# fgvieira/ngsLD

Measured on AMD Instinct MI355X. Metric: SNP-pair EM-LD computations/sec @ n_ind=500, higher is better.
Workload: dtype f64

## Files before the change

include/ngsld.h:

```cpp
#ifndef NGSLD_H
#define NGSLD_H

#include <stddef.h>
#include <stdint.h>

#ifdef __cplusplus
extern "C" {
#endif

typedef struct ngsld_ctx ngsld_ctx;

enum {
  NGSLD_OK = 0,
  NGSLD_ERR_INVALID = -1,
  NGSLD_ERR_DEVICE = -2,
  NGSLD_ERR_NOMEM = -3,
  NGSLD_ERR_NAN = -4,
  NGSLD_ERR_MAF_RANGE = -5,
  NGSLD_ERR_SINK = -6,
  NGSLD_ERR_UNSUPPORTED = -7
};

typedef struct {
  uint64_t max_kb_dist;
// ... 79 lines not shown
int ngsld_set_replay(ngsld_ctx *ctx, int enable);
int ngsld_replay_stats(ngsld_ctx *ctx, uint64_t *pairs, uint64_t *sites);

int ngsld_set_exact_store(ngsld_ctx *ctx, int mode);
typedef struct {
  uint64_t pairs_flagged;
  uint64_t pairs_replayed;
  uint64_t pairs_on_device;
  uint64_t pairs_on_host;
  uint64_t sites_reevaluated;
  int32_t exact_store;
  int32_t text_rows_patched;
  double exact_store_build_s;
  uint64_t sites_degenerate;
} ngsld_replay_stats_t;
int ngsld_replay_info(ngsld_ctx *ctx, ngsld_replay_stats_t *out);

int ngsld_run_device(ngsld_ctx *ctx, uint64_t s1_begin, uint64_t s1_end, void *d_std, void *d_ext, void *hip_stream);
int ngsld_finish_device(ngsld_ctx *ctx);

int ngsld_last_kernel_time(ngsld_ctx *ctx, double *total_ms, uint64_t *n_launches, uint64_t *n_pairs);

const char *ngsld_pair_kernel(const ngsld_ctx *ctx);
int ngsld_describe_dispatch(uint64_t n_ind, int ignore_miss_data, char *buf, size_t buf_len);

int ngsld_set_tuning(ngsld_ctx *ctx, uint32_t pairs_per_item, uint64_t batch_pairs);

int ngsld_selftest(ngsld_ctx *ctx);

int ngsld_selftest_format(ngsld_ctx *ctx, uint64_t n, const ngsld_rec_std *std, const ngsld_rec_ext *ext, const double *dist,
                          const double *maf1, const double *maf2, char *text, uint64_t text_cap, uint64_t *row_len,
                          int32_t *needs_host);
int ngsld_selftest_printed(ngsld_ctx *ctx, uint64_t n, const double *x, int32_t precision, int32_t weight_type,
                           double min_weight, int64_t *micro, int32_t *micro_ok, int64_t *label, int32_t *label_rc);

typedef struct {
  uint64_t row_begin, row_end;
  uint64_t site_end;
} ngsld_slab;

int ngsld_window_ends(const double *pos_dist, uint64_t n_sites, const ngsld_params *params, uint32_t *row_end);

int ngsld_plan_slabs(const double *pos_dist, uint64_t n_sites, const ngsld_params *params, uint64_t max_slab_sites,
                     ngsld_slab *slabs, uint64_t cap, uint64_t *n_slabs);

uint64_t ngsld_slab_sites_for_budget(uint64_t n_ind, uint64_t budget_bytes);
// ... 304 lines not shown
```

ngsld_amd/capi.py:

```python
from __future__ import annotations

import ctypes as C
import os
import subprocess

import numpy as np

PKG_DIR = os.path.dirname(os.path.abspath(__file__))
REPO_DIR = os.path.dirname(PKG_DIR)
LIB_PATH = os.environ.get("NGSLD_LIB") or os.path.join(PKG_DIR, "libngsld.so")
CLI_PATH = os.path.join(PKG_DIR, "bin", "ngsLD")

OK, ERR_INVALID, ERR_DEVICE, ERR_NOMEM, ERR_NAN, ERR_MAF_RANGE, ERR_SINK, ERR_UNSUPPORTED = 0, -1, -2, -3, -4, -5, -6, -7


class Params(C.Structure):
    _fields_ = [("max_kb_dist", C.c_uint64), ("max_snp_dist", C.c_uint64), ("min_maf", C.c_double),
                ("ignore_miss_data", C.c_int32), ("extend_out", C.c_int32), ("rnd_sample", C.c_double),
                ("seed", C.c_uint64), ("first_row", C.c_uint64)]


class GenoOpts(C.Structure):
    _fields_ = [("log_scale", C.c_int32), ("ignore_miss_data", C.c_int32), ("on_device", C.c_int32),
                ("text_semantics", C.c_int32), ("call_geno", C.c_int32), ("per_individual_only", C.c_int32),
# ... 31 lines not shown
    items = np.zeros(len(uniq), dtype=ITEM)
    items["s1"] = s1[first]
    items["s2_begin"] = s1[first] + 1 + chunk[first] * span
    items["first_record"] = first
    np.bitwise_or.at(items["mask"], inv, np.uint64(1) << (s2 - items["s2_begin"][inv]).astype(np.uint64))
    last = np.zeros(len(uniq), dtype=np.int64)
    np.maximum.at(last, inv, s2 - items["s2_begin"][inv].astype(np.int64))
    items["count"] = last + 1
    return items


SINK_FN = C.CFUNCTYPE(C.c_int, C.c_void_p, C.POINTER(Batch))
MULTI_SINK_FN = C.CFUNCTYPE(C.c_int, C.c_void_p, C.c_int, C.POINTER(Batch))
READ_FN = C.CFUNCTYPE(C.c_int, C.c_void_p, C.c_uint64, C.c_uint64, C.c_void_p)
SLAB = np.dtype([("row_begin", "<u8"), ("row_end", "<u8"), ("site_end", "<u8")])

SYMBOLS = [
    "ngsld_version", "ngsld_create", "ngsld_destroy", "ngsld_last_error", "ngsld_set_geno_raw",
    "ngsld_set_geno_raw_opts", "ngsld_set_geno_lkl",
    "ngsld_get_maf", "ngsld_set_pos_dist", "ngsld_plan", "ngsld_plan_rows", "ngsld_run", "ngsld_run_device", "ngsld_set_text_output",
    "ngsld_set_replay_source", "ngsld_set_replay_matrix", "ngsld_set_replay", "ngsld_replay_stats", "ngsld_finish_device",
    "ngsld_set_exact_store", "ngsld_replay_info",
    "ngsld_plan_parts", "ngsld_run_multi", "ngsld_multi_last_distribution", "ngsld_rccl_selftest",
    "ngsld_last_kernel_time", "ngsld_pair_kernel", "ngsld_describe_dispatch", "ngsld_set_tuning", "ngsld_selftest", "ngsld_selftest_format",
    "ngsld_selftest_printed", "ngsld_reserve_text_buffers",
    "ngsld_window_ends", "ngsld_plan_slabs", "ngsld_slab_sites_for_budget", "ngsld_sites_for_budget", "ngsld_streamed_replay_info", "ngsld_set_memory_budget", "ngsld_device_memory", "ngsld_run_streamed", "ngsld_run_streamed_text",
    "ngsld_host_read_geno_bin_range",
    "ngsld_host_set_threads", "ngsld_host_read_pos", "ngsld_host_pos_dist", "ngsld_host_label", "ngsld_host_free_pos", "ngsld_host_pos_slice",
    "ngsld_host_geno_size_ok", "ngsld_host_read_geno_bin", "ngsld_host_read_geno_text", "ngsld_host_format_header", "ngsld_host_format_pair",
    "ngsld_host_format_double", "ngsld_host_write_batch", "ngsld_host_replay_pair", "ngsld_host_missing_call_log",
    "ngsld_host_gz_open", "ngsld_host_gz_close",
    "ngsld_prune", "ngsld_host_prune_graph", "ngsld_host_prune_label",
    "ngsld_decay", "ngsld_decay_bins", "ngsld_host_decay_fit",
    "ngsld_blocks", "ngsld_blocks_sites", "ngsld_blocks_matrix", "ngsld_blocks_text",
    "ngsld_site_ld", "ngsld_site_ld_get",
    "ngsld_clusters", "ngsld_clusters_sites", "ngsld_clusters_table",
    "ngsld_grid", "ngsld_grid_cells", "ngsld_grid_chromosomes", "ngsld_grid_get",
    "ngsld_linked_pairs",
    "ngsld_scan", "ngsld_scan_get",
    "ngsld_analyze",
    "ngsld_partners", "ngsld_partners_info", "ngsld_partners_get",
]


class ReplayStats(C.Structure):
    _fields_ = [("pairs_flagged", C.c_uint64), ("pairs_replayed", C.c_uint64), ("pairs_on_device", C.c_uint64),
                ("pairs_on_host", C.c_uint64), ("sites_reevaluated", C.c_uint64), ("exact_store", C.c_int32),
# ... 186 lines not shown
        L.ngsld_get_maf.argtypes = [vp, vp]
        L.ngsld_set_pos_dist.argtypes = [vp, vp]
        L.ngsld_plan.argtypes = [vp, C.POINTER(Params), C.POINTER(u64)]
        L.ngsld_plan_rows.argtypes = [vp, C.POINTER(C.POINTER(C.c_uint64)), C.POINTER(C.POINTER(C.c_uint32))]
        L.ngsld_run.argtypes = [vp, u64, u64, SINK_FN, vp]
        L.ngsld_run_device.argtypes = [vp, u64, u64, vp, vp, vp]
        if hasattr(L, "ngsld_set_replay_source"):
            L.ngsld_set_replay_source.argtypes = [vp, READ_FN, vp]
            if hasattr(L, "ngsld_set_replay_matrix"):
                L.ngsld_set_replay_matrix.argtypes = [vp, vp]
            L.ngsld_set_replay.argtypes = [vp, C.c_int]
            L.ngsld_replay_stats.argtypes = [vp, C.POINTER(u64), C.POINTER(u64)]
        if hasattr(L, "ngsld_replay_info"):
            L.ngsld_set_exact_store.argtypes = [vp, C.c_int]
            L.ngsld_replay_info.argtypes = [vp, C.POINTER(ReplayStats)]
            L.ngsld_finish_device.argtypes = [vp]
        if hasattr(L, "ngsld_set_text_output"):
            L.ngsld_set_text_output.argtypes = [vp, C.POINTER(C.c_char_p), C.c_int]
        L.ngsld_last_kernel_time.argtypes = [vp, C.POINTER(dbl), C.POINTER(u64), C.POINTER(u64)]
        L.ngsld_set_tuning.argtypes = [vp, C.c_uint32, u64]
        if hasattr(L, "ngsld_pair_kernel"):
            L.ngsld_pair_kernel.argtypes = [vp]
            L.ngsld_pair_kernel.restype = C.c_char_p
        L.ngsld_selftest.argtypes = [vp]
        if hasattr(L, "ngsld_selftest_format"):
            L.ngsld_selftest_format.argtypes = [vp, u64, vp, vp, vp, vp, vp, C.c_char_p, u64, vp, C.POINTER(C.c_int32)]
            L.ngsld_selftest_printed.argtypes = [vp, u64, vp, C.c_int32, C.c_int32, dbl, vp, vp, vp, vp]
        L.ngsld_window_ends.argtypes = [vp, u64, C.POINTER(Params), vp]
        L.ngsld_plan_slabs.argtypes = [vp, u64, C.POINTER(Params), u64, vp, u64, C.POINTER(u64)]
        L.ngsld_slab_sites_for_budget.argtypes = [u64, u64]
        L.ngsld_slab_sites_for_budget.restype = u64
        if hasattr(L, "ngsld_sites_for_budget"):
            L.ngsld_sites_for_budget.argtypes = [u64, u64, C.c_int]
            L.ngsld_sites_for_budget.restype = u64
        L.ngsld_device_memory.argtypes = [C.c_int, C.POINTER(u64), C.POINTER(u64)]
        L.ngsld_run_streamed.argtypes = [C.c_int, u64, u64, vp, C.POINTER(Params), C.POINTER(GenoOpts), u64, READ_FN, vp,
                                         vp, SINK_FN, vp, C.POINTER(u64), C.POINTER(u64), C.c_char_p, C.c_size_t]
        if hasattr(L, "ngsld_run_multi"):
            L.ngsld_plan_parts.argtypes = [vp, u64, C.POINTER(Params), C.c_int, vp]
            L.ngsld_run_multi.argtypes = [C.POINTER(C.c_int), C.c_int, u64, u64, vp, C.POINTER(Params), C.POINTER(GenoOpts),
                                          vp, READ_FN, vp, vp, MULTI_SINK_FN, vp, C.POINTER(C.c_char_p), C.c_int,
                                          C.POINTER(u64), C.c_char_p, C.c_size_t]
        if hasattr(L, "ngsld_multi_last_distribution"):
            L.ngsld_multi_last_distribution.argtypes = []
        if hasattr(L, "ngsld_rccl_selftest"):
            L.ngsld_rccl_selftest.argtypes = [C.c_int, u64, C.c_char_p, C.c_size_t]
# ... 697 lines not shown
                fallbacks[0] += 1
            return 0

        self._check(self._L.ngsld_run(self._h, s1_begin, s1_end, SINK_FN(sink), None))
        return b"".join(parts), fallbacks[0]

    def run_discard(self, s1_begin: int = 0, s1_end: int | None = None) -> int:
        s1_end = self.n_sites if s1_end is None else s1_end
        total = [0]

        def sink(_user, bp):
            total[0] += bp.contents.n_pairs
            return 0

        self._check(self._L.ngsld_run(self._h, s1_begin, s1_end, SINK_FN(sink), None))
        return total[0]

    def run_device(self, s1_begin: int, s1_end: int, d_std: int, d_ext: int | None, stream: int | None = None) -> None:
        self._check(self._L.ngsld_run_device(self._h, s1_begin, s1_end, d_std, d_ext, stream))

    def pair_kernel(self) -> str:
        return self._L.ngsld_pair_kernel(self._h).decode()

    def last_kernel_time(self) -> tuple[float, int, int]:
        ms, nl, npairs = C.c_double(), C.c_uint64(), C.c_uint64()
        self._check(self._L.ngsld_last_kernel_time(self._h, C.byref(ms), C.byref(nl), C.byref(npairs)))
        return ms.value, nl.value, npairs.value

    def prune(self, labels: list[str] | None, field: int = 7, max_kb_dist: float = float("inf"), min_weight: float = 0.0,
              weight_type: str = "a", keep_heavy: bool = False, subset: list[str] | None = None,
              precision: int = 4) -> tuple[np.ndarray, dict]:
        return self._prune_job(labels, field, max_kb_dist, min_weight, weight_type, keep_heavy, subset, precision).run()

    def _prune_job(self, labels: list[str] | None, field: int = 7, max_kb_dist: float = float("inf"), min_weight: float = 0.0,
                   weight_type: str = "a", keep_heavy: bool = False, subset: list[str] | None = None,
                   precision: int = 4) -> _Job:
        arr = None if labels is None else (C.c_char_p * len(labels))(*[l.encode() for l in labels])
        sub = None if subset is None else (C.c_char_p * max(len(subset), 1))(*[l.encode() for l in subset])
        p = PruneParams(C.sizeof(PruneParams), field, float(max_kb_dist), float(min_weight), ord(weight_type), int(keep_heavy),
                        precision, 0, sub, 0 if subset is None else len(subset))
        st = PruneStats()
        st.struct_size = C.sizeof(PruneStats)
        state = np.zeros(max(self.n_sites, 1), dtype=np.uint8)

        def call():
            self._check(self._L.ngsld_prune(self._h, C.byref(p), arr, state.ctypes.data, C.byref(st)))
# ... 316 lines not shown
```

ngsld_amd/csrc/engine.h:

```cpp
#pragma once

#include "knobs.h"

#include <hip/hip_runtime.h>
#include <sched.h>
#include <dlfcn.h>
#include <sys/mman.h>

#include <algorithm>
#include <atomic>
#include <chrono>
#include <cmath>
#include <condition_variable>
#include <functional>
#include <cstdio>
#include <cstdlib>
#include <cstring>
#include <limits>
#include <mutex>
#include <new>
#include <string>
#include <thread>
#include <unordered_map>
#include <vector>
// ... 191 lines not shown

#include "exact_store.h"

struct FlagRow {
  uint64_t rec, off;
  uint32_t len, s1, s2, pad;
};
constexpr uint32_t kFlagRowsCap = 1024;

struct ngsld_ctx {
  int device = 0;
  hipStream_t stream = nullptr, stream2 = nullptr, copy_stream = nullptr;
  hipStream_t text_stream = nullptr;
  hipEvent_t ev_scan_done[3] = {nullptr, nullptr, nullptr};
  std::string err;

  uint64_t n_sites = 0, n_ind = 0;
  uint32_t np = 0;
  PairConfig cfg{};
  bool have_geno = false;
  DevBuf<double> d_planes, d_maf, d_mean, d_rsx, d_sc4;
  DevBuf<double> d_dose_sum;
  bool first_step_on = true;
  static constexpr int kMomentStreams = 4;
  DevBuf<double> d_moments[kMomentStreams];
  hipStream_t moments_stream[kMomentStreams] = {nullptr, nullptr, nullptr, nullptr};
  hipEvent_t moments_done[kMomentStreams] = {nullptr, nullptr, nullptr, nullptr};
  int moments_used = 0;
  DevBuf<int> d_status;
  std::vector<double> h_maf, h_pos_dist;
  DevBuf<uint64_t> d_hard_masks;
  DevBuf<double> d_hard_u;
  DevBuf<int> d_all_hard, d_odd_missing;
  int h_odd_missing = 0;
  bool missing_canonical = false;
  int h_all_hard = 0, h_prep_status = 0;
  uint32_t mask_words = 0;
  DevBuf<uint8_t> d_skip;
  DevBuf<uint32_t> d_skip_count;
  uint32_t h_skip_count = 0;
  bool skip_on = true;
  bool skip_kernels = false;

  bool planned = false;
  ngsld_params params{};
  std::vector<uint64_t> h_row_off, h_item_off;
// ... 325 lines not shown
```

ngsld_amd/csrc/engine.hip:

```cpp
#include "engine.h"

#include <atomic>

namespace ngsld {
namespace eng {

thread_local std::string g_create_error;

int set_geno_common(ngsld_ctx *c, const double *gl, const double *maf, uint64_t n_sites, uint64_t n_ind,
                    const ngsld_geno_opts &o, bool normalised) {
  if (c == nullptr) return NGSLD_ERR_INVALID;
  const int log_scale = o.log_scale, ignore_miss = o.ignore_miss_data, on_device = o.on_device;
  Range range_("ngsld:set_geno (upload + per-site prep)");
  if (o.call_geno && o.N_thresh > o.call_thresh)
    return fail(c, NGSLD_ERR_INVALID, "missing data threshold must be smaller than calling genotype threshold!");
  if (gl == nullptr || n_sites == 0 || n_ind == 0) return fail(c, NGSLD_ERR_INVALID, "empty genotype matrix");
  if (normalised && maf == nullptr) return fail(c, NGSLD_ERR_INVALID, "maf missing");
  if (n_sites >= 0xffffffffull) return fail(c, NGSLD_ERR_UNSUPPORTED, "n_sites must be below 2^32 - 1");
  PairConfig cfg;
  if (!pair_config(n_ind, &cfg, c->kernel_choice, ignore_miss != 0))
    return fail(c, NGSLD_ERR_UNSUPPORTED, "n_ind is outside the supported range");
  HIP_TRY(c, hipSetDevice(c->device));
  (void)hipGetLastError();
  {
// ... 112 lines not shown
      if (prepped[q]) (void)hipEventDestroy(prepped[q]);
    }
    if (trace) std::fprintf(stderr, "[trace] set_geno: staging buffers freed at %.2f ms\n", ms_since());
    if (rc != NGSLD_OK) return rc;
    if (e != hipSuccess) return hip_fail(c, e, "chunked genotype upload");
  }
  c->h_skip_count = 0;
  const bool look_for_skip = c->skip_on && c->replay_on && c->replay_device && c->exact_mode != 0;
  c->skip_kernels = cfg.kernel == kRun || (cfg.kernel == kMulti && cfg.form == 0 && cfg.waves == 2);
  if (look_for_skip) {
    HIP_TRY(c, c->d_skip.resize(n_sites));
    HIP_TRY(c, c->d_skip_count.resize(1));
    HIP_TRY(c, hipMemsetAsync(c->d_skip_count.p, 0, sizeof(uint32_t), c->stream));
    HIP_TRY(c, launch_site_skip(c->d_planes.p, 3ull * c->np, c->np, (uint32_t)n_ind, ignore_miss, c->d_maf.p, n_sites, c->d_skip.p,
                                c->d_skip_count.p, c->stream));
    HIP_TRY(c, hipMemcpyAsync(&c->h_skip_count, c->d_skip_count.p, sizeof(uint32_t), hipMemcpyDeviceToHost, c->stream));
  } else {
    c->d_skip.release();
  }
  HIP_TRY(c, launch_pack_scalars(c->d_maf.p, c->d_mean.p, c->d_rsx.p, c->d_skip.p, c->d_sc4.p, n_sites, c->stream));
  if (cfg.kernel == kRun && !ignore_miss && cfg.slots >= 2 && cfg.slots <= 8) {
    c->first_step_on = !test_knob_is("FIRST_STEP", "0");
    HIP_TRY(c, c->d_dose_sum.resize(n_sites));
    HIP_TRY(c, launch_site_dose(c->d_planes.p, 3ull * c->np, c->np, (uint32_t)n_ind, c->d_maf.p, c->d_skip.p, n_sites, c->d_dose_sum.p,
                                c->stream));
  } else {
    c->d_dose_sum.release();
  }
  int &all_hard = c->h_all_hard;
  all_hard = 0;
  const char *hk = test_knob("HARD_KERNEL");
  const bool try_hard = n_ind <= kHardMaxInd && !o.per_individual_only && !(hk != nullptr && std::strcmp(hk, "0") == 0);
  if (try_hard) {
    c->mask_words = (uint32_t)((n_ind + 63) / 64);
    HIP_TRY(c, c->d_hard_masks.resize((size_t)n_sites * 4 * c->mask_words));
    HIP_TRY(c, c->d_hard_u.resize(n_sites));
    HIP_TRY(c, c->d_all_hard.resize(1));
    all_hard = 1;
    HIP_TRY(c, hipMemcpyAsync(c->d_all_hard.p, &all_hard, sizeof(int), hipMemcpyHostToDevice, c->stream));
    HIP_TRY(c, launch_classify_hard(c->d_planes.p, 3ull * c->np, c->np, (uint32_t)n_ind, n_sites, c->d_hard_masks.p,
                                    c->d_hard_u.p, c->d_all_hard.p, c->stream));
    HIP_TRY(c, hipMemcpyAsync(&all_hard, c->d_all_hard.p, sizeof(int), hipMemcpyDeviceToHost, c->stream));
    if (trace) std::fprintf(stderr, "[trace] set_geno: called-genotype check enqueued at %.2f ms\n", ms_since());
  }
  c->h_maf.resize(n_sites);
  int &status = c->h_prep_status;
  status = 0;
  HIP_TRY(c, hipMemcpyAsync(c->h_maf.data(), c->d_maf.p, n_sites * sizeof(double), hipMemcpyDeviceToHost, c->stream));
  HIP_TRY(c, hipMemcpyAsync(&status, c->d_status.p, sizeof(int), hipMemcpyDeviceToHost, c->stream));
  c->h_odd_missing = 1;
  if (look_for_odd_missing)
    HIP_TRY(c, hipMemcpyAsync(&c->h_odd_missing, c->d_odd_missing.p, sizeof(int), hipMemcpyDeviceToHost, c->stream));
  HIP_TRY(c, hipStreamSynchronize(c->stream));
  c->missing_canonical = look_for_odd_missing && c->h_odd_missing == 0;
  if (trace) std::fprintf(stderr, "[trace] set_geno: scalars packed, called-genotype check, maf on the host at %.2f ms\n", ms_since());
  if (status == NGSLD_ERR_NAN) return fail(c, NGSLD_ERR_NAN, "NaN found! Is the file format correct?");
  if (try_hard && all_hard) {
    c->cfg.kernel = kHard;
    c->cfg.group = 16;
    c->cfg.slots = 1;
    c->cfg.waves = 1;
    c->d_dose_sum.release();
  } else {
    c->d_hard_masks.release();
    c->d_hard_u.release();
  }
  c->have_geno = true;
  return NGSLD_OK;
}
}
}

extern "C" {

const char *ngsld_version(void) { return "ngsld-amd 0.15.0 (gfx950; reference ngsLD 1.2.1)"; }

int ngsld_create(int device, ngsld_ctx **out) {
  if (out == nullptr) return NGSLD_ERR_INVALID;
  *out = nullptr;
  int n_dev = 0;
  hipError_t e = hipGetDeviceCount(&n_dev);
  if (e != hipSuccess || n_dev == 0) {
    g_create_error = std::string("no HIP device available (") + hipGetErrorString(e) +
                     "); this library has no CPU fallback";
    return NGSLD_ERR_DEVICE;
  }
  if (device < 0 || device >= n_dev) {
    g_create_error = "device index out of range";
    return NGSLD_ERR_INVALID;
  }
  hipDeviceProp_t prop;
  e = hipGetDeviceProperties(&prop, device);
  if (e != hipSuccess) {
    g_create_error = std::string("hipGetDeviceProperties: ") + hipGetErrorString(e);
    return NGSLD_ERR_DEVICE;
  }
  if (std::strncmp(prop.gcnArchName, "gfx950", 6) != 0) {
    g_create_error = std::string("device is ") + prop.gcnArchName + ", this build targets gfx950 (MI355X) only";
// ... 24 lines not shown
  if (const char *k = test_knob("RUN_DIRECT")) c->run_direct = std::strcmp(k, "0") != 0;
  if (const char *k = test_knob("RUN_TAPER")) c->run_taper = std::strcmp(k, "0") != 0;
  if (const char *k = test_knob("RUN_STREAMS")) c->run_streams = std::atoi(k) >= 2 ? 2 : 1;
  if ((e = hipSetDevice(device)) != hipSuccess || (e = hipStreamCreate(&c->stream)) != hipSuccess ||
      (e = hipStreamCreate(&c->stream2)) != hipSuccess || (e = hipStreamCreate(&c->copy_stream)) != hipSuccess) {
    g_create_error = std::string("stream setup: ") + hipGetErrorString(e);
    delete c;
    return NGSLD_ERR_DEVICE;
  }
  for (int k = 0; k < ngsld_ctx::kSlots; ++k) {
    (void)hipEventCreateWithFlags(&c->ev_kernel_done[k], hipEventDisableTiming);
    (void)hipEventCreateWithFlags(&c->ev_copy_done[k], hipEventDisableTiming);
  }
  *out = c;
  return NGSLD_OK;
}

void ngsld_destroy(ngsld_ctx *c) {
  if (c == nullptr) return;
  if (c->reserve_thread.joinable()) c->reserve_thread.join();
  c->store.destroy();
  (void)hipSetDevice(c->device);
  (void)hipDeviceSynchronize();
  c->d_planes.release(); c->d_maf.release(); c->d_mean.release(); c->d_rsx.release(); c->d_sc4.release(); c->d_dose_sum.release(); c->d_runs.release(); c->d_skip.release(); c->d_skip_count.release();
  for (auto &b : c->d_moments) b.release();
  for (auto &e : c->moments_done)
    if (e) (void)hipEventDestroy(e);
  c->d_hard_masks.release(); c->d_hard_u.release(); c->d_all_hard.release();
  c->lane_scratch_dev.release();
  for (int k = 0; k < ngsld_ctx::kSlots; ++k) c->lane_scratch[k].release();
  c->d_labels.release(); c->d_scan_tmp.release(); c->d_scan_tmp_b.release(); c->d_label_off.release(); c->d_cum.release(); c->d_infc.release();
  for (int k = 0; k < ngsld_ctx::kSlots; ++k) {
    c->d_text[k].release(); c->d_lens[k].release(); c->d_offs[k].release(); c->d_text_meta[k].release();
    c->h_text[k].release(); c->h_text_meta[k].release();
  }
  c->d_status.release(); c->d_row_off.release(); c->d_item_off.release(); c->d_row_end.release();
  c->d_row_seed.release(); c->d_row_count.release(); c->d_keep.release(); c->d_items.release();
  for (int k = 0; k < ngsld_ctx::kSlots; ++k) {
    c->d_std[k].release(); c->d_ext[k].release(); c->h_std[k].release(); c->h_ext[k].release();
    if (c->ev_kernel_done[k]) (void)hipEventDestroy(c->ev_kernel_done[k]);
    if (c->ev_copy_done[k]) (void)hipEventDestroy(c->ev_copy_done[k]);
  }
  for (auto &ev : c->ev_pool) {
    (void)hipEventDestroy(ev.first);
    (void)hipEventDestroy(ev.second);
  }
  if (c->stream) (void)hipStreamDestroy(c->stream);
// ... 39 lines not shown

int ngsld_set_pos_dist(ngsld_ctx *c, const double *pos_dist) try {
  if (c == nullptr) return NGSLD_ERR_INVALID;
  if (!c->have_geno) return fail(c, NGSLD_ERR_INVALID, "set the genotype data before the positions");
  c->planned = false;
  c->clear_blocks();
  if (pos_dist == nullptr)
    c->h_pos_dist.assign(c->n_sites, std::numeric_limits<double>::infinity());
  else
    c->h_pos_dist.assign(pos_dist, pos_dist + c->n_sites);
  return NGSLD_OK;
} NGSLD_CATCH(c)
const char *ngsld_pair_kernel(const ngsld_ctx *c) {
  if (c == nullptr || !c->have_geno) return "";
  switch (effective_kernel(c->cfg, c->params.ignore_miss_data != 0)) {
    case kGroup: return "group";
    case kMulti: return c->cfg.form == 1 ? "multi-ab" : "multi";
    case kStream: return "stream";
    case kRun: return "run";
    case kHard: return "hard";
    case kRunAB: return "ab";
    default: return "";
  }
}

int ngsld_describe_dispatch(uint64_t n_ind, int ignore_miss_data, char *buf, size_t buf_len) {
  if (buf == nullptr || buf_len == 0) return NGSLD_ERR_INVALID;
  buf[0] = 0;
  PairConfig cfg;
  const bool masked = ignore_miss_data != 0;
  if (!pair_config(n_ind, &cfg, kChooseAuto, masked)) return NGSLD_ERR_UNSUPPORTED;
  const char *family = "";
  int slots = cfg.slots, waves = cfg.waves;
  switch (effective_kernel(cfg, masked)) {
    case kGroup: family = "group"; break;
    case kMulti:
      family = cfg.form == 1 ? "multi-ab" : "multi";
      if (cfg.form == 0) multi_shape(cfg, masked, &slots, &waves);
      break;
    case kStream: family = "stream"; break;
    case kRun: family = "run"; break;
    case kRunAB: family = "ab"; break;
    default: return NGSLD_ERR_UNSUPPORTED;
  }
  const int n = std::snprintf(buf, buf_len, "%s %dx%d lanes=%d np=%u", family, waves, slots, cfg.group, cfg.np);
  return (n < 0 || (size_t)n >= buf_len) ? NGSLD_ERR_INVALID : NGSLD_OK;
// ... 203 lines not shown
```

ngsld_amd/csrc/engine_plan.hip:

```cpp
#include "engine.h"

namespace ngsld {
namespace eng {

void plan_rows(const std::vector<double> &pos_dist, const std::vector<double> &maf, const ngsld_params &p,
               uint64_t n, std::vector<uint32_t> &row_end) {
  row_end.assign(n, 0);
  const bool use_dist = p.max_kb_dist > 0;
  const double limit = (double)(p.max_kb_dist * 1000);
  bool exact = true;
  std::vector<double> cum;
  std::vector<uint32_t> seg;
  if (use_dist) {
    cum.assign(n, 0.0);
    seg.assign(n, 0);
    double run = 0.0;
    uint32_t sg = 0;
    for (uint64_t s = 0; s < n; ++s) {
      const double g = pos_dist[s];
      if (std::isinf(g) && g > 0) {
        if (s > 0) ++sg;
      } else if (s > 0) {
        if (!(g >= 1.0) || g != std::floor(g) || run + g > 9.0e15) exact = false;
        run += g;
// ... 97 lines not shown
  c->replayed_sites = 0;
  if (c->replay_on && (c->replay_read != nullptr || c->replay_matrix != nullptr) && !c->normalised) {
    bool changed = false;
    std::vector<double> tmp;
    ReplaySite site;
    for (uint64_t s = 0; s < n; ++s) {
      const double m = c->h_maf[s], t = std::fabs(m) * 1e6;
      const bool tie = p->min_maf > 0 && std::fabs(m - p->min_maf) <= 1e-12;
      const bool edge = p->extend_out && std::fabs((t - std::floor(t)) - 0.5) < 1e-6;
      if (!tie && !edge) continue;
      const int rcs = fetch_replay_site(c, s, tmp, &site);
      if (rcs != NGSLD_OK) return fail(c, rcs, "the replay source callback failed");
      ++c->replayed_sites;
      if (site.maf != m && !(site.maf != site.maf && m != m)) {
        c->h_maf[s] = site.maf;
        changed = true;
      }
    }
    if (changed) {
      HIP_TRY(c, hipMemcpy(c->d_maf.p, c->h_maf.data(), n * sizeof(double), hipMemcpyHostToDevice));
      HIP_TRY(c, launch_pack_scalars(c->d_maf.p, c->d_mean.p, c->d_rsx.p, c->d_skip.p, c->d_sc4.p, n, c->stream));
      if (c->d_dose_sum.p != nullptr)
        HIP_TRY(c, launch_site_dose(c->d_planes.p, 3ull * c->np, c->np, (uint32_t)c->n_ind, c->d_maf.p, c->d_skip.p, n, c->d_dose_sum.p,
                                    c->stream));
    }
  }
  plan_rows(c->h_pos_dist, c->h_maf, *p, n, c->h_row_end);
  c->h_keep.resize(n);
  for (uint64_t s = 0; s < n; ++s) c->h_keep[s] = (c->h_maf[s] < p->min_maf) ? 0 : 1;
  const uint64_t ch = item_span(c->cfg, c->pairs_per_item);
  c->h_item_off.resize(n + 1);
  c->h_item_off[0] = 0;
  for (uint64_t s1 = 0; s1 < n; ++s1) {
    const uint64_t end = c->h_row_end[s1];
    const uint64_t span = end > s1 + 1 ? end - (s1 + 1) : 0;
    c->h_item_off[s1 + 1] = c->h_item_off[s1] + (span + ch - 1) / ch;
  }
  c->n_items = c->h_item_off[n];
  if (uses_runs(c->cfg.kernel)) {
    if (c->n_items > 0xffffffffull) return fail(c, NGSLD_ERR_UNSUPPORTED, "more than 2^32 work items in one plan");
    c->run_len = 0;
  }
  HIP_TRY(c, c->d_row_end.resize(n));
  HIP_TRY(c, c->d_keep.resize(n));
  HIP_TRY(c, c->d_row_off.resize(n + 1));
  HIP_TRY(c, c->d_item_off.resize(n + 1));
  HIP_TRY(c, c->d_row_count.resize(n));
// ... 72 lines not shown
```

ngsld_amd/csrc/engine_run.hip:

```cpp
#include "engine.h"
#include "../../include/ngsld_host.h"

namespace ngsld {
namespace eng {

static hipError_t launch_run_with_moments(ngsld_ctx *c, const PairArgs &a, hipStream_t stream) {
  const std::vector<uint64_t> &ro = c->h_row_off;
  const uint64_t total = ro[a.row1] - ro[a.row0];
  if (total == 0) return hipSuccess;
  uint64_t longest = 0;
  for (uint64_t r = a.row0; r < a.row1; ++r) longest = std::max(longest, ro[r + 1] - ro[r]);
  int k = 0;
  while (k < c->moments_used && c->moments_stream[k] != stream) ++k;
  if (k == c->moments_used) {
    if (k == ngsld_ctx::kMomentStreams) {
      k = ngsld_ctx::kMomentStreams - 1;
      const hipError_t e = hipEventSynchronize(c->moments_done[k]);
      if (e != hipSuccess) return e;
    } else {
      ++c->moments_used;
      const hipError_t e = hipEventCreateWithFlags(&c->moments_done[k], hipEventDisableTiming);
      if (e != hipSuccess) {
        --c->moments_used;
        return e;
// ... 16 lines not shown
      cap = grow;
    }
  }
  cap = std::min(cap, want);
  const bool masked = false;
  for (uint64_t r0 = a.row0; r0 < a.row1;) {
    const uint64_t r1 = rows_within(ro, r0, a.row1, cap);
    if (ro[r1] > ro[r0]) {
      MomentArgs m{};
      m.planes = a.planes;
      m.site_stride = a.site_stride;
      m.np = a.np;
      m.n_ind = a.n_ind;
      m.maf = a.maf;
      m.n_sites = c->n_sites;
      m.items_all = a.items_all;
      m.item_off = a.item_off;
      m.row_end = c->d_row_end.p;
      m.row0 = (uint32_t)r0;
      m.row1 = (uint32_t)r1;
      m.dose = (a.dose_sum != nullptr && c->cfg.slots >= 2 && c->cfg.slots <= 8) ? 1 : 0;
      m.rec0 = ro[r0];
      m.out = buf.p;
      hipError_t e = launch_pair_moments(m, c->h_row_end.data(), stream);
      if (e != hipSuccess) return e;
      PairArgs b = a;
      b.row0 = (uint32_t)r0;
      b.row1 = (uint32_t)r1;
      b.items = c->d_items.p + c->h_item_off[r0];
      b.n_items = c->h_item_off[r1] - c->h_item_off[r0];
      b.runs = c->d_runs.p + c->h_run_off[r0];
      b.n_runs = c->h_run_off[r1] - c->h_run_off[r0];
      b.moments = reinterpret_cast<const double *>(reinterpret_cast<uintptr_t>(buf.p) - 16 * (ro[r0] - a.out_base));
      e = launch_pair_kernel(c->cfg, masked, b, stream);
      if (e != hipSuccess) return e;
    }
    r0 = r1;
  }
  return hipEventRecord(c->moments_done[k], stream);
}

hipError_t timed_launch(ngsld_ctx *c, const PairArgs &a, hipStream_t stream) {
  if (c->ev_used == c->ev_pool.size()) {
    hipEvent_t b, e;
    hipError_t r = hipEventCreate(&b);
    if (r != hipSuccess) return r;
// ... 954 lines not shown
```

ngsld_amd/csrc/ld_dispatch.h:

```cpp
#pragma once

#include "ld_common.h"

namespace ngsld {

constexpr int kBresMinSlots = 11, kBresMaxSlots = 20;
constexpr int kBresTailSlots = 20;

enum PairKernel { kGroup = 0, kMulti = 2, kStream = 4, kRun = 5, kHard = 6, kRunAB = 7 };
enum PairChoice { kChooseAuto = 0, kChooseMulti = 1, kChooseAB = 2, kChoosePlainStream = 3, kChooseABMulti = 4, kChooseResidentStream = 5 };
inline bool uses_runs(int kernel) { return kernel == kRun || kernel == kGroup || kernel == kHard || kernel == kRunAB; }
constexpr uint32_t kHardMaxWords = 512;
constexpr uint64_t kHardMaxInd = 64ull * kHardMaxWords;
struct PairConfig {
  int kernel;
  int group;
  int slots;
  int waves;
  int form;
  uint32_t np;
};
bool pair_config(uint64_t n_ind, PairConfig *cfg, int choice = kChooseAuto, bool masked = false);
inline int effective_kernel(const PairConfig &cfg, bool ) { return cfg.kernel; }
inline void multi_shape(const PairConfig &cfg, bool masked, int *slots, int *waves) {
// ... 4 lines not shown
    *waves = 4;
  }
}
hipError_t launch_pair_kernel(const PairConfig &cfg, bool masked, const PairArgs &args, hipStream_t stream);
hipError_t launch_pair_hard(bool masked, const PairArgs &args, hipStream_t stream);
hipError_t launch_pair_ab(int slots, bool masked, const PairArgs &args, hipStream_t stream);
hipError_t launch_pair_abm(int slots, int waves, bool masked, const PairArgs &args, hipStream_t stream);
hipError_t launch_pair_bres(int slots, bool masked, const PairArgs &args, hipStream_t stream);
hipError_t launch_classify_hard(const double *planes, uint64_t site_stride, uint32_t np, uint32_t n_ind, uint64_t n_sites,
                                uint64_t *masks, double *u, int *all_hard, hipStream_t stream);
struct MomentArgs {
  const double *planes;
  uint64_t site_stride;
  uint32_t np, n_ind;
  const double *maf;
  uint64_t n_sites;
  const Item *items_all;
  const uint64_t *item_off;
  const uint32_t *row_end;
  uint32_t row0, row1;
  uint32_t dose;
  uint64_t rec0;
  double *out;
};
hipError_t launch_pair_moments(const MomentArgs &args, const uint32_t *h_row_end, hipStream_t stream);
inline uint32_t item_span(const PairConfig &cfg, uint32_t pairs_per_item) {
  if (uses_runs(cfg.kernel)) return 64u;
  const uint32_t span = cfg.kernel == kMulti ? 4u * pairs_per_item : pairs_per_item;
  return span > 64u ? 64u : span;
}

}
```

ngsld_amd/csrc/ld_pair_moments.hip:

```cpp
#include <algorithm>

#include "ld_dispatch.h"

namespace ngsld {

namespace {
constexpr uint32_t kTR = 128, kTC = 64, kKc = 16;
constexpr uint32_t kSites = kTR + kTC;
constexpr uint32_t kLd = kSites + 16;
typedef double v4d __attribute__((ext_vector_type(4)));
typedef double v2d __attribute__((ext_vector_type(2)));
}

template <bool DOSE>
__global__ __launch_bounds__(512) void pair_ld_moments_kernel(MomentArgs A) {
  __shared__ double sE[kKc * kLd];
  __shared__ double sD[DOSE ? kKc * kLd : 1];
  __shared__ uint64_t s_ioff[kTR];
  __shared__ uint32_t s_end[kTR];
  __shared__ uint32_t s_cmax;
  const uint32_t t = threadIdx.x, lane = t & 63u;
  const uint32_t wave = (uint32_t)__builtin_amdgcn_readfirstlane((int)(t >> 6));
  const uint32_t rb = A.row0 + blockIdx.y * kTR;
  const uint64_t c0 = (uint64_t)rb + 1u + (uint64_t)blockIdx.x * kTC;
  if (t == 0) s_cmax = 0;
  __syncthreads();
  if (t < kTR) {
    const uint32_t row = rb + t;
    const bool in = row < A.row1;
    const uint32_t e = in ? A.row_end[row] : 0u;
    s_end[t] = e;
    s_ioff[t] = in ? A.item_off[row] : 0ull;
    atomicMax(&s_cmax, e);
  }
  __syncthreads();
  const uint32_t cmax = s_cmax;
  if (c0 >= cmax) return;

  const bool loader = t < 2 * kSites;
  const uint32_t sl = t < kSites ? t : (loader ? t - kSites : 0u), half = t < kSites ? 0u : 1u;
  uint64_t site = sl < kTR ? (uint64_t)rb + sl : c0 + (sl - kTR);
  if (site >= A.n_sites) site = A.n_sites - 1;
  const double m = A.maf[site];
  const bool flip = m > 0.5;
  const DoseWeights u = dose_weights(flip ? 1.0 - m : m);
  const double *pl = A.planes + site * A.site_stride + half * 8u;
  const double *p0 = pl + (flip ? 2u * A.np : 0u), *p1 = pl + A.np, *p2 = pl + (flip ? 0u : 2u * A.np);
  v2d q0[4], q1[4], q2[4];
  auto fetch = [&](uint32_t kc) {
#pragma unroll
    for (int i = 0; i < 4; ++i) {
      q0[i] = reinterpret_cast<const v2d *>(p0 + kc * kKc)[i];
      q1[i] = reinterpret_cast<const v2d *>(p1 + kc * kKc)[i];
      q2[i] = reinterpret_cast<const v2d *>(p2 + kc * kKc)[i];
    }
  };
  auto stage = [&](uint32_t kc) {
#pragma unroll
    for (int i = 0; i < 8; ++i) {
      const double a0 = q0[i >> 1][i & 1], a1 = q1[i >> 1][i & 1], a2 = q2[i >> 1][i & 1];
      const uint32_t k = half * 8u + (uint32_t)i;
      sE[k * kLd + sl] = fma(2.0, a2, a1);
      if (DOSE) {
        double den, num;
        dose_terms(u, a0, a1, a2, den, num);
        sD[k * kLd + sl] = kc * kKc + k < A.n_ind ? num / den : 0.0;
      }
    }
  };

  const uint32_t wr = wave & 3u, wc = wave >> 2;
  bool live[2][2];
#pragma unroll
  for (int ri = 0; ri < 2; ++ri)
#pragma unroll
    for (int cj = 0; cj < 2; ++cj) {
      const uint64_t r_lo = (uint64_t)rb + wr * 32u + ri * 16u, c_lo = c0 + wc * 32u + cj * 16u;
      live[ri][cj] = r_lo < A.row1 && c_lo + 15u > r_lo && c_lo < cmax;
    }
  v4d totE[2][2], totD[2][2];
#pragma unroll
  for (int ri = 0; ri < 2; ++ri)
#pragma unroll
    for (int cj = 0; cj < 2; ++cj) totE[ri][cj] = totD[ri][cj] = v4d{0.0, 0.0, 0.0, 0.0};
// ... 58 lines not shown
        if (!(mask & bit)) continue;
        const uint64_t idx = it->first_record + (uint64_t)__popcll(mask & (bit - 1)) - A.rec0;
        reinterpret_cast<v2d *>(A.out)[idx] = v2d{totE[ri][cj][r], DOSE ? totD[ri][cj][r] : 0.0};
      }
    }
}

hipError_t launch_pair_moments(const MomentArgs &a, const uint32_t *h_row_end, hipStream_t stream) {
  if (a.row1 <= a.row0) return hipSuccess;
  uint64_t most = 0;
  for (uint32_t rb = a.row0; rb < a.row1; rb += kTR) {
    uint32_t end = 0;
    for (uint32_t r = rb; r < a.row1 && r < rb + kTR; ++r) end = std::max(end, h_row_end[r]);
    if (end > rb + 1) most = std::max<uint64_t>(most, ((uint64_t)end - rb - 1 + kTC - 1) / kTC);
  }
  if (most == 0) return hipSuccess;
  if (most > (1ull << 22)) return hipErrorInvalidValue;
  const uint64_t blocks_y = std::min<uint64_t>(65535, std::max<uint64_t>(1, (1ull << 22) / most));
  for (uint64_t r0 = a.row0; r0 < a.row1; r0 += blocks_y * kTR) {
    MomentArgs b = a;
    b.row0 = (uint32_t)r0;
    const uint64_t by = std::min<uint64_t>(blocks_y, ((uint64_t)a.row1 - r0 + kTR - 1) / kTR);
    const dim3 grid((unsigned)most, (unsigned)by), block(512);
    if (a.dose)
      hipLaunchKernelGGL((pair_ld_moments_kernel<true>), grid, block, 0, stream, b);
    else
      hipLaunchKernelGGL((pair_ld_moments_kernel<false>), grid, block, 0, stream, b);
    const hipError_t e = hipGetLastError();
    if (e != hipSuccess) return e;
  }
  return hipSuccess;
}

}
```

ngsld_amd/csrc/ld_prep.h:

```cpp
#pragma once

#include "ld_common.h"

namespace ngsld {

struct PrepArgs {
  const double *raw;
  uint64_t site0;
  const double *maf_in;
  double *planes;
  uint64_t site_stride;
  uint64_t n_sites;
  uint32_t np, n_ind;
  int log_scale, ignore_miss, normalised_input;
  int text_semantics, call_geno;
  int exact_chain;
  double N_thresh, call_thresh;
  double *maf, *mean_e, *rsx;
  int *status;
  int *odd_missing;
  double missing_canon;
};

hipError_t launch_prep(const PrepArgs &a, hipStream_t stream);
struct ItemArgs {
  const uint32_t *row_end;
  const uint8_t *keep;
  const uint64_t *row_seed;
  const uint64_t *row_off;
  const uint64_t *item_off;
  uint64_t *row_count;
  Item *items;
  uint32_t n_sites, span;
  double rnd_sample;
  int count_only;
};
hipError_t launch_items(const ItemArgs &a, hipStream_t stream);
hipError_t launch_pack_scalars(const double *maf, const double *mean_e, const double *rsx, const uint8_t *skip, double *sc4, uint64_t n,
                               hipStream_t stream);
hipError_t launch_site_skip(const double *planes, uint64_t site_stride, uint32_t np, uint32_t n_ind, int ignore_miss, const double *maf,
                            uint64_t n_sites, uint8_t *skip, uint32_t *count, hipStream_t stream);
hipError_t launch_site_dose(const double *planes, uint64_t site_stride, uint32_t np, uint32_t n_ind, const double *maf, const uint8_t *skip,
                            uint64_t n_sites, double *dose_sum, hipStream_t stream);
hipError_t launch_selftest(const double *in, double *out, hipStream_t stream);

}
```

ngsld_amd/csrc/ld_prep.hip:

```cpp
#include "ld_prep.h"
#include "taus.h"

namespace ngsld {

__device__ __forceinline__ double logsum3(double g0, double g1, double g2) {
  double M = g0;
  M = g1 >= M ? g1 : M;
  M = g2 >= M ? g2 : M;
  if (M == -__builtin_inf()) return -__builtin_inf();
  double sum = 0.0;
  sum += exp(g0 - M);
  sum += exp(g1 - M);
  sum += exp(g2 - M);
  return log(sum) + M;
}

__device__ __forceinline__ double conv_log(double g) {
  g = log(g);
  return g == -__builtin_inf() ? -1e15 : g;
}

__device__ __forceinline__ void call_geno(double &g0, double &g1, double &g2, double N_thresh, double call_thresh) {
  int max_pos = 0;
  double mx = -__builtin_inf();
// ... 387 lines not shown
    hipLaunchKernelGGL(site_skip_kernel<0>, grid, block, 0, stream, planes, site_stride, np, n_ind, ignore_miss, maf, n_sites, skip, count);
  return hipGetLastError();
}

__global__ void pack_scalars_kernel(const double *maf, const double *mean_e, const double *rsx, const uint8_t *skip, double *sc4, uint64_t n) {
  const uint64_t s = (uint64_t)blockIdx.x * blockDim.x + threadIdx.x;
  if (s >= n) return;
  sc4[4 * s] = maf[s];
  sc4[4 * s + 1] = mean_e[s];
  sc4[4 * s + 2] = rsx[s];
  sc4[4 * s + 3] = (skip != nullptr && skip[s]) ? 1.0 : 0.0;
}

hipError_t launch_pack_scalars(const double *maf, const double *mean_e, const double *rsx, const uint8_t *skip, double *sc4, uint64_t n,
                               hipStream_t stream) {
  if (n == 0) return hipSuccess;
  hipLaunchKernelGGL(pack_scalars_kernel, dim3((unsigned)((n + 255) / 256)), dim3(256), 0, stream, maf, mean_e, rsx, skip, sc4, n);
  return hipGetLastError();
}

constexpr double kDoseDenMin = 0x1p-500;
__global__ __launch_bounds__(256) void site_dose_kernel(const double *__restrict__ planes, uint64_t site_stride, uint32_t np, uint32_t n_ind,
                                                        const double *__restrict__ maf, const uint8_t *__restrict__ skip, uint64_t n_sites,
                                                        double *__restrict__ dose_sum) {
  const int lane = threadIdx.x & 63, wave = threadIdx.x >> 6;
  for (uint64_t site = (uint64_t)blockIdx.x * 4 + wave; site < n_sites; site += (uint64_t)gridDim.x * 4) {
    const double *pl = planes + site * site_stride;
    const double m_in = maf[site];
    const bool flip = m_in > 0.5;
    const double m = flip ? 1.0 - m_in : m_in;
    const DoseWeights u = dose_weights(m);
    const double *p0 = pl + (flip ? 2ull * np : 0ull), *p1 = pl + np, *p2 = pl + (flip ? 0ull : 2ull * np);
    bool ok = m_in > 0.0 && m_in < 1.0;
    const bool marked = skip != nullptr && skip[site];
    double acc = 0.0, prod = 1.0;
    for (uint32_t i = (uint32_t)lane; i < n_ind; i += 64) {
      const double a0 = p0[i], a1 = p1[i], a2 = p2[i];
      double den, num;
      dose_terms(u, a0, a1, a2, den, num);
      const double d = num / den;
      ok = ok && den >= kDoseDenMin && den < __builtin_inf() && d >= 0.0 && d < __builtin_inf() && !odd_triple(a0, a1, a2);
      acc += d;
      prod *= den;
    }
    ok = ok && prod >= kDoseDenMin * kDoseDenMin;
    const double S = wave_sum1(acc);
    const bool all_ok = __ballot(!ok) == 0 && S >= 0.0 && S < __builtin_inf();
    if (lane == 0) dose_sum[site] = all_ok ? (marked ? -2.0 : S) : -1.0;
  }
}

hipError_t launch_site_dose(const double *planes, uint64_t site_stride, uint32_t np, uint32_t n_ind, const double *maf, const uint8_t *skip,
                            uint64_t n_sites, double *dose_sum, hipStream_t stream) {
  if (n_sites == 0) return hipSuccess;
  const uint64_t wgs = (n_sites + 3) / 4;
  hipLaunchKernelGGL(site_dose_kernel, dim3((unsigned)(wgs < 65536 ? wgs : 65536)), dim3(256), 0, stream, planes, site_stride, np, n_ind, maf,
                     skip, n_sites, dose_sum);
  return hipGetLastError();
}

__global__ void items_kernel(ItemArgs A) {
  const uint32_t s1 = blockIdx.x * blockDim.x + threadIdx.x;
  if (s1 >= A.n_sites) return;
  const uint32_t end = A.row_end[s1];
  const bool sampling = A.row_seed != nullptr;
  Taus rng;
  if (sampling) rng.set(A.row_seed[s1]);
  uint64_t kept = 0;
  uint64_t k = A.count_only ? 0 : A.item_off[s1];
  const uint64_t base = A.count_only ? 0 : A.row_off[s1];
  for (uint32_t b = s1 + 1; b < end; b += A.span) {
    const uint32_t cnt = end - b < A.span ? end - b : A.span;
    uint64_t mask = 0;
    for (uint32_t c = 0; c < cnt; ++c) {
      if (!A.keep[b + c]) continue;
      if (sampling && rng.uniform() > A.rnd_sample) continue;
      mask |= 1ull << c;
    }
    if (!A.count_only) {
      Item it;
// ... 46 lines not shown
```

Baseline: 213.9 million.

## Precompute per-site expected-genotype and dose vectors for the pair moments kernel

The site dose prep kernel now also writes, for each site, a compact vector of expected genotype (2*a2+a1) and dose values (padded to np). The pair moments kernel gets a VEC template path that loads these two precomputed planes instead of three likelihood planes, and skips the per-pair flip, dose_weights and dose_terms arithmetic during staging. This cuts global reads and redundant per-tile arithmetic, at the cost of extra device memory (2*np doubles per site) and a larger prep pass. It is gated by a memory check and a test knob.

```diff
diff --git a/include/ngsld.h b/include/ngsld.h
--- a/include/ngsld.h
+++ b/include/ngsld.h
@@ -125,6 +125,7 @@
 int ngsld_last_kernel_time(ngsld_ctx *ctx, double *total_ms, uint64_t *n_launches, uint64_t *n_pairs);
 
 const char *ngsld_pair_kernel(const ngsld_ctx *ctx);
+uint64_t ngsld_site_vector_bytes(const ngsld_ctx *ctx);
 int ngsld_describe_dispatch(uint64_t n_ind, int ignore_miss_data, char *buf, size_t buf_len);
 
 int ngsld_set_tuning(ngsld_ctx *ctx, uint32_t pairs_per_item, uint64_t batch_pairs);
diff --git a/ngsld_amd/capi.py b/ngsld_amd/capi.py
--- a/ngsld_amd/capi.py
+++ b/ngsld_amd/capi.py
@@ -77,7 +77,7 @@
     "ngsld_set_replay_source", "ngsld_set_replay_matrix", "ngsld_set_replay", "ngsld_replay_stats", "ngsld_finish_device",
     "ngsld_set_exact_store", "ngsld_replay_info",
     "ngsld_plan_parts", "ngsld_run_multi", "ngsld_multi_last_distribution", "ngsld_rccl_selftest",
-    "ngsld_last_kernel_time", "ngsld_pair_kernel", "ngsld_describe_dispatch", "ngsld_set_tuning", "ngsld_selftest", "ngsld_selftest_format",
+    "ngsld_last_kernel_time", "ngsld_pair_kernel", "ngsld_site_vector_bytes", "ngsld_describe_dispatch", "ngsld_set_tuning", "ngsld_selftest", "ngsld_selftest_format",
     "ngsld_selftest_printed", "ngsld_reserve_text_buffers",
     "ngsld_window_ends", "ngsld_plan_slabs", "ngsld_slab_sites_for_budget", "ngsld_sites_for_budget", "ngsld_streamed_replay_info", "ngsld_set_memory_budget", "ngsld_device_memory", "ngsld_run_streamed", "ngsld_run_streamed_text",
     "ngsld_host_read_geno_bin_range",
@@ -310,6 +310,9 @@
         if hasattr(L, "ngsld_pair_kernel"):
             L.ngsld_pair_kernel.argtypes = [vp]
             L.ngsld_pair_kernel.restype = C.c_char_p
+        if hasattr(L, "ngsld_site_vector_bytes"):
+            L.ngsld_site_vector_bytes.argtypes = [vp]
+            L.ngsld_site_vector_bytes.restype = u64
         L.ngsld_selftest.argtypes = [vp]
         if hasattr(L, "ngsld_selftest_format"):
             L.ngsld_selftest_format.argtypes = [vp, u64, vp, vp, vp, vp, vp, C.c_char_p, u64, vp, C.POINTER(C.c_int32)]
@@ -1053,6 +1056,9 @@
     def pair_kernel(self) -> str:
         return self._L.ngsld_pair_kernel(self._h).decode()
 
+    def site_vector_bytes(self) -> int:
+        return int(self._L.ngsld_site_vector_bytes(self._h))
+
     def last_kernel_time(self) -> tuple[float, int, int]:
         ms, nl, npairs = C.c_double(), C.c_uint64(), C.c_uint64()
         self._check(self._L.ngsld_last_kernel_time(self._h, C.byref(ms), C.byref(nl), C.byref(npairs)))
diff --git a/ngsld_amd/csrc/engine.h b/ngsld_amd/csrc/engine.h
--- a/ngsld_amd/csrc/engine.h
+++ b/ngsld_amd/csrc/engine.h
@@ -237,6 +237,7 @@
   DevBuf<double> d_planes, d_maf, d_mean, d_rsx, d_sc4;
   DevBuf<double> d_dose_sum;
   bool first_step_on = true;
+  DevBuf<double> d_site_vec;
   static constexpr int kMomentStreams = 4;
   DevBuf<double> d_moments[kMomentStreams];
   hipStream_t moments_stream[kMomentStreams] = {nullptr, nullptr, nullptr, nullptr};
diff --git a/ngsld_amd/csrc/engine.hip b/ngsld_amd/csrc/engine.hip
--- a/ngsld_amd/csrc/engine.hip
+++ b/ngsld_amd/csrc/engine.hip
@@ -158,10 +158,16 @@
   if (cfg.kernel == kRun && !ignore_miss && cfg.slots >= 2 && cfg.slots <= 8) {
     c->first_step_on = !test_knob_is("FIRST_STEP", "0");
     HIP_TRY(c, c->d_dose_sum.resize(n_sites));
+    const uint64_t vec_elems = (uint64_t)n_sites * 2 * c->np;
+    if (test_knob_is("SITE_VECTORS", "0") || (c->d_site_vec.n < vec_elems && !room_for(vec_elems * sizeof(double), 8ull << 30, 1ull << 30)))
+      c->d_site_vec.release();
+    else
+      HIP_TRY(c, c->d_site_vec.resize(vec_elems));
     HIP_TRY(c, launch_site_dose(c->d_planes.p, 3ull * c->np, c->np, (uint32_t)n_ind, c->d_maf.p, c->d_skip.p, n_sites, c->d_dose_sum.p,
-                                c->stream));
+                                c->d_site_vec.p, c->stream));
   } else {
     c->d_dose_sum.release();
+    c->d_site_vec.release();
   }
   int &all_hard = c->h_all_hard;
   all_hard = 0;
@@ -197,6 +203,7 @@
     c->cfg.slots = 1;
     c->cfg.waves = 1;
     c->d_dose_sum.release();
+    c->d_site_vec.release();
   } else {
     c->d_hard_masks.release();
     c->d_hard_u.release();
@@ -209,7 +216,7 @@
 
 extern "C" {
 
-const char *ngsld_version(void) { return "ngsld-amd 0.15.0 (gfx950; reference ngsLD 1.2.1)"; }
+const char *ngsld_version(void) { return "ngsld-amd 0.15.1 (gfx950; reference ngsLD 1.2.1)"; }
 
 int ngsld_create(int device, ngsld_ctx **out) {
   if (out == nullptr) return NGSLD_ERR_INVALID;
@@ -280,7 +287,7 @@
   c->store.destroy();
   (void)hipSetDevice(c->device);
   (void)hipDeviceSynchronize();
-  c->d_planes.release(); c->d_maf.release(); c->d_mean.release(); c->d_rsx.release(); c->d_sc4.release(); c->d_dose_sum.release(); c->d_runs.release(); c->d_skip.release(); c->d_skip_count.release();
+  c->d_planes.release(); c->d_maf.release(); c->d_mean.release(); c->d_rsx.release(); c->d_sc4.release(); c->d_dose_sum.release(); c->d_site_vec.release(); c->d_runs.release(); c->d_skip.release(); c->d_skip_count.release();
   for (auto &b : c->d_moments) b.release();
   for (auto &e : c->moments_done)
     if (e) (void)hipEventDestroy(e);
@@ -366,6 +373,10 @@
     case kRunAB: return "ab";
     default: return "";
   }
+}
+
+uint64_t ngsld_site_vector_bytes(const ngsld_ctx *c) {
+  return (c == nullptr || !c->have_geno || c->d_site_vec.p == nullptr) ? 0 : (uint64_t)c->n_sites * 2 * c->np * sizeof(double);
 }
 
 int ngsld_describe_dispatch(uint64_t n_ind, int ignore_miss_data, char *buf, size_t buf_len) {
diff --git a/ngsld_amd/csrc/engine_plan.hip b/ngsld_amd/csrc/engine_plan.hip
--- a/ngsld_amd/csrc/engine_plan.hip
+++ b/ngsld_amd/csrc/engine_plan.hip
@@ -143,7 +143,7 @@
       HIP_TRY(c, launch_pack_scalars(c->d_maf.p, c->d_mean.p, c->d_rsx.p, c->d_skip.p, c->d_sc4.p, n, c->stream));
       if (c->d_dose_sum.p != nullptr)
         HIP_TRY(c, launch_site_dose(c->d_planes.p, 3ull * c->np, c->np, (uint32_t)c->n_ind, c->d_maf.p, c->d_skip.p, n, c->d_dose_sum.p,
-                                    c->stream));
+                                    c->d_site_vec.p, c->stream));
     }
   }
   plan_rows(c->h_pos_dist, c->h_maf, *p, n, c->h_row_end);
diff --git a/ngsld_amd/csrc/engine_run.hip b/ngsld_amd/csrc/engine_run.hip
--- a/ngsld_amd/csrc/engine_run.hip
+++ b/ngsld_amd/csrc/engine_run.hip
@@ -62,6 +62,7 @@
       m.dose = (a.dose_sum != nullptr && c->cfg.slots >= 2 && c->cfg.slots <= 8) ? 1 : 0;
       m.rec0 = ro[r0];
       m.out = buf.p;
+      m.site_vec = c->d_site_vec.p;
       hipError_t e = launch_pair_moments(m, c->h_row_end.data(), stream);
       if (e != hipSuccess) return e;
       PairArgs b = a;
diff --git a/ngsld_amd/csrc/ld_dispatch.h b/ngsld_amd/csrc/ld_dispatch.h
--- a/ngsld_amd/csrc/ld_dispatch.h
+++ b/ngsld_amd/csrc/ld_dispatch.h
@@ -50,6 +50,7 @@
   uint32_t dose;
   uint64_t rec0;
   double *out;
+  const double *site_vec;
 };
 hipError_t launch_pair_moments(const MomentArgs &args, const uint32_t *h_row_end, hipStream_t stream);
 inline uint32_t item_span(const PairConfig &cfg, uint32_t pairs_per_item) {
diff --git a/ngsld_amd/csrc/ld_pair_moments.hip b/ngsld_amd/csrc/ld_pair_moments.hip
--- a/ngsld_amd/csrc/ld_pair_moments.hip
+++ b/ngsld_amd/csrc/ld_pair_moments.hip
@@ -12,7 +12,7 @@
 typedef double v2d __attribute__((ext_vector_type(2)));
 }
 
-template <bool DOSE>
+template <bool DOSE, bool VEC>
 __global__ __launch_bounds__(512) void pair_ld_moments_kernel(MomentArgs A) {
   __shared__ double sE[kKc * kLd];
   __shared__ double sD[DOSE ? kKc * kLd : 1];
@@ -41,25 +41,30 @@
   const uint32_t sl = t < kSites ? t : (loader ? t - kSites : 0u), half = t < kSites ? 0u : 1u;
   uint64_t site = sl < kTR ? (uint64_t)rb + sl : c0 + (sl - kTR);
   if (site >= A.n_sites) site = A.n_sites - 1;
-  const double m = A.maf[site];
+  const double m = VEC ? 0.0 : A.maf[site];
   const bool flip = m > 0.5;
   const DoseWeights u = dose_weights(flip ? 1.0 - m : m);
-  const double *pl = A.planes + site * A.site_stride + half * 8u;
-  const double *p0 = pl + (flip ? 2u * A.np : 0u), *p1 = pl + A.np, *p2 = pl + (flip ? 0u : 2u * A.np);
+  const double *pl = VEC ? A.site_vec + site * 2u * A.np + half * 8u : A.planes + site * A.site_stride + half * 8u;
+  const double *p0 = pl + (VEC ? A.np : (flip ? 2u * A.np : 0u)), *p1 = VEC ? pl : pl + A.np, *p2 = pl + (flip ? 0u : 2u * A.np);
   v2d q0[4], q1[4], q2[4];
   auto fetch = [&](uint32_t kc) {
 #pragma unroll
     for (int i = 0; i < 4; ++i) {
-      q0[i] = reinterpret_cast<const v2d *>(p0 + kc * kKc)[i];
+      if (!VEC || DOSE) q0[i] = reinterpret_cast<const v2d *>(p0 + kc * kKc)[i];
       q1[i] = reinterpret_cast<const v2d *>(p1 + kc * kKc)[i];
-      q2[i] = reinterpret_cast<const v2d *>(p2 + kc * kKc)[i];
+      if (!VEC) q2[i] = reinterpret_cast<const v2d *>(p2 + kc * kKc)[i];
     }
   };
   auto stage = [&](uint32_t kc) {
 #pragma unroll
     for (int i = 0; i < 8; ++i) {
+      const uint32_t k = half * 8u + (uint32_t)i;
+      if (VEC) {
+        sE[k * kLd + sl] = q1[i >> 1][i & 1];
+        if (DOSE) sD[k * kLd + sl] = q0[i >> 1][i & 1];
+        continue;
+      }
       const double a0 = q0[i >> 1][i & 1], a1 = q1[i >> 1][i & 1], a2 = q2[i >> 1][i & 1];
-      const uint32_t k = half * 8u + (uint32_t)i;
       sE[k * kLd + sl] = fma(2.0, a2, a1);
       if (DOSE) {
         double den, num;
@@ -164,10 +169,16 @@
     b.row0 = (uint32_t)r0;
     const uint64_t by = std::min<uint64_t>(blocks_y, ((uint64_t)a.row1 - r0 + kTR - 1) / kTR);
     const dim3 grid((unsigned)most, (unsigned)by), block(512);
-    if (a.dose)
-      hipLaunchKernelGGL((pair_ld_moments_kernel<true>), grid, block, 0, stream, b);
-    else
-      hipLaunchKernelGGL((pair_ld_moments_kernel<false>), grid, block, 0, stream, b);
+    if (a.site_vec != nullptr) {
+      if (a.dose)
+        hipLaunchKernelGGL((pair_ld_moments_kernel<true, true>), grid, block, 0, stream, b);
+      else
+        hipLaunchKernelGGL((pair_ld_moments_kernel<false, true>), grid, block, 0, stream, b);
+    } else if (a.dose) {
+      hipLaunchKernelGGL((pair_ld_moments_kernel<true, false>), grid, block, 0, stream, b);
+    } else {
+      hipLaunchKernelGGL((pair_ld_moments_kernel<false, false>), grid, block, 0, stream, b);
+    }
     const hipError_t e = hipGetLastError();
     if (e != hipSuccess) return e;
   }
diff --git a/ngsld_amd/csrc/ld_prep.h b/ngsld_amd/csrc/ld_prep.h
--- a/ngsld_amd/csrc/ld_prep.h
+++ b/ngsld_amd/csrc/ld_prep.h
@@ -41,7 +41,7 @@
 hipError_t launch_site_skip(const double *planes, uint64_t site_stride, uint32_t np, uint32_t n_ind, int ignore_miss, const double *maf,
                             uint64_t n_sites, uint8_t *skip, uint32_t *count, hipStream_t stream);
 hipError_t launch_site_dose(const double *planes, uint64_t site_stride, uint32_t np, uint32_t n_ind, const double *maf, const uint8_t *skip,
-                            uint64_t n_sites, double *dose_sum, hipStream_t stream);
+                            uint64_t n_sites, double *dose_sum, double *site_vec, hipStream_t stream);
 hipError_t launch_selftest(const double *in, double *out, hipStream_t stream);
 
 }
diff --git a/ngsld_amd/csrc/ld_prep.hip b/ngsld_amd/csrc/ld_prep.hip
--- a/ngsld_amd/csrc/ld_prep.hip
+++ b/ngsld_amd/csrc/ld_prep.hip
@@ -433,7 +433,7 @@
 constexpr double kDoseDenMin = 0x1p-500;
 __global__ __launch_bounds__(256) void site_dose_kernel(const double *__restrict__ planes, uint64_t site_stride, uint32_t np, uint32_t n_ind,
                                                         const double *__restrict__ maf, const uint8_t *__restrict__ skip, uint64_t n_sites,
-                                                        double *__restrict__ dose_sum) {
+                                                        double *__restrict__ dose_sum, double *__restrict__ site_vec) {
   const int lane = threadIdx.x & 63, wave = threadIdx.x >> 6;
   for (uint64_t site = (uint64_t)blockIdx.x * 4 + wave; site < n_sites; site += (uint64_t)gridDim.x * 4) {
     const double *pl = planes + site * site_stride;
@@ -445,11 +445,17 @@
     bool ok = m_in > 0.0 && m_in < 1.0;
     const bool marked = skip != nullptr && skip[site];
     double acc = 0.0, prod = 1.0;
-    for (uint32_t i = (uint32_t)lane; i < n_ind; i += 64) {
+    double *ve = site_vec != nullptr ? site_vec + site * 2ull * np : nullptr;
+    for (uint32_t i = (uint32_t)lane; i < (ve != nullptr ? np : n_ind); i += 64) {
       const double a0 = p0[i], a1 = p1[i], a2 = p2[i];
       double den, num;
       dose_terms(u, a0, a1, a2, den, num);
       const double d = num / den;
+      if (ve != nullptr) {
+        ve[i] = fma(2.0, a2, a1);
+        ve[np + i] = i < n_ind ? d : 0.0;
+      }
+      if (i >= n_ind) continue;
       ok = ok && den >= kDoseDenMin && den < __builtin_inf() && d >= 0.0 && d < __builtin_inf() && !odd_triple(a0, a1, a2);
       acc += d;
       prod *= den;
@@ -462,11 +468,11 @@
 }
 
 hipError_t launch_site_dose(const double *planes, uint64_t site_stride, uint32_t np, uint32_t n_ind, const double *maf, const uint8_t *skip,
-                            uint64_t n_sites, double *dose_sum, hipStream_t stream) {
+                            uint64_t n_sites, double *dose_sum, double *site_vec, hipStream_t stream) {
   if (n_sites == 0) return hipSuccess;
   const uint64_t wgs = (n_sites + 3) / 4;
   hipLaunchKernelGGL(site_dose_kernel, dim3((unsigned)(wgs < 65536 ? wgs : 65536)), dim3(256), 0, stream, planes, site_stride, np, n_ind, maf,
-                     skip, n_sites, dose_sum);
+                     skip, n_sites, dose_sum, site_vec);
   return hipGetLastError();
 }
 
```

New measurement: 215.0 million, median of 5. About the same (+0.5%).
